# gsgen3d/gsgen

Measured on AMD Instinct MI355X. Metric: fwd+bwd renders/sec (800x800, 100k Gaussians), higher is better.
Workload: dtype f32

## Files before the change

gsgen_amd/csrc/geometry.hip:

```cpp
#include <string.h>

#include "common.hpp"
#include "../../include/gsgen_hip.h"

namespace gs {

constexpr int kThreads = 256;

__device__ __forceinline__ bool sphere_in_frustum(float mx, float my, float mz, float r,
                                                  const float *__restrict__ normal,
                                                  const float *__restrict__ pts) {
  bool ok = true;
#pragma unroll
  for (int k = 0; k < 6; ++k) {
    const float d = (mx - pts[3 * k]) * normal[3 * k] + (my - pts[3 * k + 1]) * normal[3 * k + 1] +
                    (mz - pts[3 * k + 2]) * normal[3 * k + 2];
    ok = ok && (d > -r);
  }
  return ok;
}

__global__ void __launch_bounds__(kThreads)
k_cull_bsphere(uint32_t N, const float *__restrict__ mean, const float *__restrict__ svec,
               const float *__restrict__ normal, const float *__restrict__ pts,
               uint8_t *__restrict__ mask, float thresh) {
  const uint32_t i = blockIdx.x * blockDim.x + threadIdx.x;
  if (i >= N) return;
  const float r = fmaxf(fmaxf(svec[3 * i], svec[3 * i + 1]), svec[3 * i + 2]) * thresh;
  mask[i] = sphere_in_frustum(mean[3 * i], mean[3 * i + 1], mean[3 * i + 2], r, normal, pts) ? 1 : 0;
}

struct Proj {
  float m2x, m2y, c00, c01, c10, c11, depth;
  float A[9];
};

__device__ __forceinline__ void quat_to_rot(const float *__restrict__ q, float *R) {
  float n = sqrtf(q[0] * q[0] + q[1] * q[1] + q[2] * q[2] + q[3] * q[3]);
  n = fmaxf(n, 1e-12f);
  const float w = q[0] / n, x = q[1] / n, y = q[2] / n, z = q[3] / n;
  const float tx = 2.0f * x, ty = 2.0f * y, tz = 2.0f * z;
  const float twx = tx * w, twy = ty * w, twz = tz * w;
  const float txx = tx * x, txy = ty * x, txz = tz * x;
  const float tyy = ty * y, tyz = tz * y, tzz = tz * z;
  R[0] = 1.0f - (tyy + tzz); R[1] = txy - twz;          R[2] = txz + twy;
  R[3] = txy + twz;          R[4] = 1.0f - (txx + tzz); R[5] = tyz - twx;
  R[6] = txz - twy;          R[7] = tyz + twx;          R[8] = 1.0f - (txx + tyy);
}

__device__ __forceinline__ Proj project_one(const float *__restrict__ p, const float *__restrict__ q,
                                            const float *__restrict__ s, const float *Rc,
                                            const float *t) {
  Proj o;
  const float d0 = p[0] - t[0], d1 = p[1] - t[1], d2 = p[2] - t[2];
  float u[3];
#pragma unroll
  for (int i = 0; i < 3; ++i) u[i] = Rc[i] * d0 + Rc[3 + i] * d1 + Rc[6 + i] * d2;
  float Rq[9];
  quat_to_rot(q, Rq);
  float M[9];
#pragma unroll
  for (int i = 0; i < 3; ++i)
#pragma unroll
    for (int j = 0; j < 3; ++j) M[i * 3 + j] = s[j] * Rq[i * 3 + j];
  float S[9];
#pragma unroll
  for (int i = 0; i < 3; ++i)
#pragma unroll
    for (int k = 0; k < 3; ++k)
      S[i * 3 + k] = M[i * 3] * M[k * 3] + M[i * 3 + 1] * M[k * 3 + 1] + M[i * 3 + 2] * M[k * 3 + 2];
  const float x = u[0], y = u[1], z = u[2];
  const float l = sqrtf(x * x + y * y + z * z);
  const float J[9] = {1.0f / z, 0.0f, -x / z / z, 0.0f, 1.0f / z, -y / z / z, x / l, y / l, z / l};
#pragma unroll
  for (int i = 0; i < 3; ++i)
#pragma unroll
    for (int k = 0; k < 3; ++k)
      o.A[i * 3 + k] = J[i * 3] * Rc[k * 3] + J[i * 3 + 1] * Rc[k * 3 + 1] + J[i * 3 + 2] * Rc[k * 3 + 2];
  float T1[6];
#pragma unroll
  for (int a = 0; a < 2; ++a)
#pragma unroll
    for (int k = 0; k < 3; ++k)
      T1[a * 3 + k] = o.A[a * 3] * S[k] + o.A[a * 3 + 1] * S[3 + k] + o.A[a * 3 + 2] * S[6 + k];
  o.c00 = T1[0] * o.A[0] + T1[1] * o.A[1] + T1[2] * o.A[2];
  o.c01 = T1[0] * o.A[3] + T1[1] * o.A[4] + T1[2] * o.A[5];
  o.c10 = T1[3] * o.A[0] + T1[4] * o.A[1] + T1[5] * o.A[2];
  o.c11 = T1[3] * o.A[3] + T1[4] * o.A[4] + T1[5] * o.A[5];
  o.depth = z;
  o.m2x = x / z;
  o.m2y = y / z;
  return o;
}

__device__ __forceinline__ void load_pose(const float *__restrict__ c2w, float *Rc, float *t) {
#pragma unroll
  for (int i = 0; i < 3; ++i) {
#pragma unroll
    for (int j = 0; j < 3; ++j) Rc[i * 3 + j] = c2w[i * 4 + j];
    t[i] = c2w[i * 4 + 3];
  }
}

__global__ void __launch_bounds__(kThreads)
k_project(uint32_t N, const float *__restrict__ mean, const float *__restrict__ qvec,
          const float *__restrict__ svec, const float *__restrict__ c2w, float *__restrict__ mean2d,
          float *__restrict__ cov2d, float *__restrict__ JW, float *__restrict__ depth) {
  const uint32_t i = blockIdx.x * blockDim.x + threadIdx.x;
  if (i >= N) return;
  float Rc[9], t[3];
  load_pose(c2w, Rc, t);
  const Proj o = project_one(mean + 3 * (size_t)i, qvec + 4 * (size_t)i, svec + 3 * (size_t)i, Rc, t);
  *reinterpret_cast<float2 *>(mean2d + 2 * (size_t)i) = make_float2(o.m2x, o.m2y);
  *reinterpret_cast<float4 *>(cov2d + 4 * (size_t)i) = make_float4(o.c00, o.c01, o.c10, o.c11);
  depth[i] = o.depth;
  if (JW != nullptr) {
#pragma unroll
    for (int k = 0; k < 9; ++k) JW[9 * (size_t)i + k] = o.A[k];
  }
}

constexpr int kAdamMaxGroups = 8;
struct AdamArgs {
  uint64_t end[kAdamMaxGroups];
  float step_size[kAdamMaxGroups];
  uint32_t n_groups;
  float bc2_sqrt, beta1, beta2, eps;
  const float *dev;
};

__global__ void __launch_bounds__(kThreads)
k_adam_step(uint64_t n, float *__restrict__ param, const float *__restrict__ grad,
            float *__restrict__ exp_avg, float *__restrict__ exp_avg_sq, AdamArgs a) {
  const uint64_t i0 = 4 * ((uint64_t)blockIdx.x * blockDim.x + threadIdx.x);
  if (i0 >= n) return;
  const float w1 = 1.0f - a.beta1, w2 = 1.0f - a.beta2;
  if (a.dev != nullptr) {
#pragma unroll
    for (int k = 0; k < kAdamMaxGroups; ++k) a.step_size[k] = a.dev[k];
    a.bc2_sqrt = a.dev[kAdamMaxGroups];
  }
#pragma unroll
  for (int e = 0; e < 4; ++e) {
    const uint64_t i = i0 + e;
    if (i >= n) break;
    float ss = a.step_size[0];
#pragma unroll
    for (int k = 1; k < kAdamMaxGroups; ++k)
      if (k < (int)a.n_groups && i >= a.end[k - 1]) ss = a.step_size[k];
    const float g = grad[i];
    float m = exp_avg[i], v = exp_avg_sq[i];
    m = m + (g - m) * w1;
    v = v * a.beta2 + (w2 * g) * g;
    const float denom = sqrtf(v) / a.bc2_sqrt + a.eps;
    param[i] = param[i] - ss * (m / denom);
    exp_avg[i] = m;
    exp_avg_sq[i] = v;
  }
}

__global__ void __launch_bounds__(kThreads)
k_densify_update(uint32_t N, const float *__restrict__ cov2d, const float *__restrict__ g_mean2d,
                 const uint8_t *__restrict__ mask, float *__restrict__ max_radii2d,
                 float *__restrict__ grad_accum, float *__restrict__ cnt) {
  const uint32_t n = blockIdx.x * blockDim.x + threadIdx.x;
  if (n >= N) return;
  if (mask != nullptr && mask[n] == 0) return;
  if (max_radii2d != nullptr) {
    const float4 c = *reinterpret_cast<const float4 *>(cov2d + 4 * (size_t)n);
    const float m = (c.x + c.w) / 2.0f;
    const float det = c.x * c.w - c.y * c.z;
    const float r = m + sqrtf(fmaxf(m * m - det, 0.0f));
    if (!(r < 0.0f)) atomicMax(reinterpret_cast<unsigned int *>(max_radii2d) + n, __float_as_uint(r));
  }
  if (grad_accum != nullptr) {
    const float2 g = *reinterpret_cast<const float2 *>(g_mean2d + 2 * (size_t)n);
    atomicAdd(grad_accum + n, sqrtf(g.x * g.x + g.y * g.y));
    if (cnt != nullptr) atomicAdd(cnt + n, 1.0f);
  }
}

constexpr int kStatViews = 16;
struct DensifyViews {
  const float *cov2d[kStatViews], *g_mean2d[kStatViews];
  const uint8_t *mask[kStatViews];
};
__global__ void __launch_bounds__(kThreads)
k_densify_update_views(uint32_t N, DensifyViews dv, int n_views, float *__restrict__ max_radii2d,
                       float *__restrict__ grad_accum, float *__restrict__ cnt) {
  const uint32_t n = blockIdx.x * blockDim.x + threadIdx.x;
  if (n >= N) return;
  float rmax = 0.0f, gsum = 0.0f, visits = 0.0f;
  bool seen = false, rnan = false;
  for (int v = 0; v < n_views; ++v) {
    const uint8_t *m = dv.mask[v];
    if (m != nullptr && m[n] == 0) continue;
    seen = true;
    if (max_radii2d != nullptr) {
      const float4 c = *reinterpret_cast<const float4 *>(dv.cov2d[v] + 4 * (size_t)n);
      const float mm = (c.x + c.w) / 2.0f;
      const float det = c.x * c.w - c.y * c.z;
      const float r = mm + sqrtf(fmaxf(mm * mm - det, 0.0f));
      if (r != r) rnan = true;
      else rmax = fmaxf(rmax, r);
    }
    if (grad_accum != nullptr) {
      const float2 g = *reinterpret_cast<const float2 *>(dv.g_mean2d[v] + 2 * (size_t)n);
      gsum += sqrtf(g.x * g.x + g.y * g.y);
      visits += 1.0f;
    }
  }
  if (!seen) return;
  if (max_radii2d != nullptr)
    atomicMax(reinterpret_cast<unsigned int *>(max_radii2d) + n,
              rnan ? 0x7fc00000u : __float_as_uint(rmax));
  if (grad_accum != nullptr) {
    atomicAdd(grad_accum + n, gsum);
    if (cnt != nullptr) atomicAdd(cnt + n, visits);
  }
}

struct ProjGrad { float gm[3], gq[4], gs[3]; };
struct CholK { double k0, k1, k2; };
__device__ __forceinline__ CholK chol_k_of(const float *__restrict__ cov2d_n) {
  const CholRec c = chol_prep(cov2d_n[0], cov2d_n[1], cov2d_n[2], cov2d_n[3]);
  CholK k{0.0, 0.0, 0.0};
  if (c.ok) { k.k0 = (double)kInvSc2 * (double)c.p0; k.k1 = (double)kInvSc2 * (double)c.p1; k.k2 = (double)kInvSc2 * (double)c.p2; }
  return k;
}
__device__ __forceinline__ ProjGrad project_bwd_one(uint32_t n, const float *__restrict__ mean,
                                                    const float *__restrict__ qvec, const float *__restrict__ svec,
                                                    const float *__restrict__ c2w, int detach_depth,
                                                    double gm0, double gm1, const double (&gc)[4], float g_depth_n) {
#pragma clang fp contract(fast)
  ProjGrad o;
  double Rc[9], t[3];
#pragma unroll
  for (int i = 0; i < 3; ++i) {
#pragma unroll
    for (int j = 0; j < 3; ++j) Rc[i * 3 + j] = (double)c2w[i * 4 + j];
    t[i] = (double)c2w[i * 4 + 3];
  }
  const float *p = mean + 3 * (size_t)n, *q = qvec + 4 * (size_t)n, *sf = svec + 3 * (size_t)n;
  const double s[3] = {(double)sf[0], (double)sf[1], (double)sf[2]};
  const double d0 = (double)p[0] - t[0], d1 = (double)p[1] - t[1], d2 = (double)p[2] - t[2];
  double u[3];
#pragma unroll
  for (int i = 0; i < 3; ++i) u[i] = Rc[i] * d0 + Rc[3 + i] * d1 + Rc[6 + i] * d2;
  double nq = sqrt((double)q[0] * q[0] + (double)q[1] * q[1] + (double)q[2] * q[2] + (double)q[3] * q[3]);
  nq = nq < 1e-12 ? 1e-12 : nq;
  const double inq = 1.0 / nq;
  const double w = q[0] * inq, x = q[1] * inq, y = q[2] * inq, z = q[3] * inq;
  const double Rq[9] = {1 - 2 * (y * y + z * z), 2 * (x * y - w * z), 2 * (x * z + w * y),
                        2 * (x * y + w * z), 1 - 2 * (x * x + z * z), 2 * (y * z - w * x),
                        2 * (x * z - w * y), 2 * (y * z + w * x), 1 - 2 * (x * x + y * y)};
  double M[9];
#pragma unroll
  for (int i = 0; i < 3; ++i)
#pragma unroll
    for (int j = 0; j < 3; ++j) M[i * 3 + j] = s[j] * Rq[i * 3 + j];
  const double ux = u[0], uy = u[1], uz = u[2];
  const double iz = 1.0 / uz;
  const double j02 = -ux * iz * iz, j12 = -uy * iz * iz;
  double A[6];
#pragma unroll
  for (int k = 0; k < 3; ++k) {
    A[k] = iz * Rc[k * 3] + j02 * Rc[k * 3 + 2];
    A[3 + k] = iz * Rc[k * 3 + 1] + j12 * Rc[k * 3 + 2];
  }
  double GA[6];
#pragma unroll
  for (int k = 0; k < 3; ++k) {
    GA[k] = gc[0] * A[k] + gc[1] * A[3 + k];
    GA[3 + k] = gc[2] * A[k] + gc[3] * A[3 + k];
  }
  double dS[9];
#pragma unroll
  for (int j = 0; j < 3; ++j)
#pragma unroll
    for (int k = 0; k < 3; ++k) dS[j * 3 + k] = A[j] * GA[k] + A[3 + j] * GA[3 + k];
  double dM[9];
#pragma unroll
  for (int i = 0; i < 3; ++i)
#pragma unroll
    for (int j = 0; j < 3; ++j) {
      double acc = 0.0;
#pragma unroll
      for (int k = 0; k < 3; ++k) acc += (dS[i * 3 + k] + dS[k * 3 + i]) * M[k * 3 + j];
      dM[i * 3 + j] = acc;
    }
  double dR[9];
#pragma unroll
  for (int j = 0; j < 3; ++j) {
    double acc = 0.0;
#pragma unroll
    for (int i = 0; i < 3; ++i) {
      acc += dM[i * 3 + j] * Rq[i * 3 + j];
      dR[i * 3 + j] = dM[i * 3 + j] * s[j];
    }
    o.gs[j] = (float)acc;
  }
  double dq[4];
  dq[0] = 2 * (-z * dR[1] + y * dR[2] + z * dR[3] - x * dR[5] - y * dR[6] + x * dR[7]);
  dq[1] = 2 * (y * dR[1] + z * dR[2] + y * dR[3] - 2 * x * dR[4] - w * dR[5] + z * dR[6] + w * dR[7] - 2 * x * dR[8]);
  dq[2] = 2 * (-2 * y * dR[0] + x * dR[1] + w * dR[2] + x * dR[3] + z * dR[5] - w * dR[6] + z * dR[7] - 2 * y * dR[8]);
  dq[3] = 2 * (-2 * z * dR[0] - w * dR[1] + x * dR[2] + w * dR[3] - 2 * z * dR[4] + y * dR[5] + x * dR[6] + y * dR[7]);
  const double qh[4] = {w, x, y, z};
  const double dot = qh[0] * dq[0] + qh[1] * dq[1] + qh[2] * dq[2] + qh[3] * dq[3];
#pragma unroll
  for (int k = 0; k < 4; ++k) o.gq[k] = (float)((dq[k] - qh[k] * dot) * inq);
  double du[3] = {gm0 * iz, gm1 * iz, (double)g_depth_n};
  if (!detach_depth) du[2] += -(ux * gm0 + uy * gm1) * iz * iz;
#pragma unroll
  for (int j = 0; j < 3; ++j) o.gm[j] = (float)(Rc[j * 3] * du[0] + Rc[j * 3 + 1] * du[1] + Rc[j * 3 + 2] * du[2]);
  return o;
}
__device__ __forceinline__ ProjGrad project_bwd_one(uint32_t n, const float *__restrict__ mean,
                                                    const float *__restrict__ qvec, const float *__restrict__ svec,
                                                    const float *__restrict__ c2w, int detach_depth,
                                                    const float *__restrict__ g_mean2d,
                                                    const float *__restrict__ g_cov2d, float g_depth_n) {
  const float4 g = *reinterpret_cast<const float4 *>(g_cov2d + 4 * (size_t)n);
  const double gc[4] = {(double)g.x, (double)g.y, (double)g.z, (double)g.w};
  return project_bwd_one(n, mean, qvec, svec, c2w, detach_depth, (double)g_mean2d[2 * (size_t)n],
                         (double)g_mean2d[2 * (size_t)n + 1], gc, g_depth_n);
}

template <bool ACC>
__global__ void __launch_bounds__(kThreads)
k_project_bwd(uint32_t N, const float *__restrict__ mean, const float *__restrict__ qvec,
              const float *__restrict__ svec, const float *__restrict__ c2w, int detach_depth,
              const uint8_t *__restrict__ mask, const float *__restrict__ g_mean2d,
              const float *__restrict__ g_cov2d, const float *__restrict__ g_depth,
              float *__restrict__ g_mean, float *__restrict__ g_qvec, float *__restrict__ g_svec) {
  const uint32_t n = blockIdx.x * blockDim.x + threadIdx.x;
  if (n >= N) return;
  float *gm = g_mean + 3 * (size_t)n, *gq = g_qvec + 4 * (size_t)n, *gs_ = g_svec + 3 * (size_t)n;
  if (mask != nullptr && mask[n] == 0) {
    if constexpr (!ACC) {
      gm[0] = gm[1] = gm[2] = 0.f;
      gq[0] = gq[1] = gq[2] = gq[3] = 0.f;
      gs_[0] = gs_[1] = gs_[2] = 0.f;
    }
    return;
  }
  auto put = [](float *dst, float v) {
    if constexpr (ACC) atomicAdd(dst, v);
    else *dst = v;
  };
  const ProjGrad o = project_bwd_one(n, mean, qvec, svec, c2w, detach_depth, g_mean2d, g_cov2d,
                                     g_depth != nullptr ? g_depth[n] : 0.0f);
#pragma unroll
  for (int j = 0; j < 3; ++j) put(gs_ + j, o.gs[j]);
#pragma unroll
  for (int k = 0; k < 4; ++k) put(gq + k, o.gq[k]);
#pragma unroll
  for (int j = 0; j < 3; ++j) put(gm + j, o.gm[j]);
}

constexpr int kProjViews = 16;
struct ProjBwdViews {
  const float *cam[kProjViews];
  const uint8_t *mask[kProjViews];
  const float *g_mean2d[kProjViews], *g_cov2d[kProjViews], *g_depth[kProjViews];
  const float *g_chan6[kProjViews], *depth[kProjViews];
  const float *cov2d[kProjViews];
  const float *chol[kProjViews];
};
__device__ __forceinline__ void moments_to_grads(const CholK &k, const float *__restrict__ mom2, const float *__restrict__ mom4,
                                                 double &gm0, double &gm1, double (&gc)[4]) {
  const double Mu = (double)mom2[0], Mv = (double)mom2[1];
  const double Muu = (double)mom4[0], Muv = (double)mom4[1], Mvv = (double)mom4[2];
  gm0 = k.k0 * Mu;
  gm1 = k.k1 * Mu + k.k2 * Mv;
  gc[0] = 0.5 * k.k0 * k.k0 * Muu;
  gc[1] = gc[2] = 0.5 * k.k0 * (k.k1 * Muu + k.k2 * Muv);
  gc[3] = 0.5 * (k.k1 * k.k1 * Muu + 2.0 * k.k1 * k.k2 * Muv + k.k2 * k.k2 * Mvv);
}
__device__ __forceinline__ void moments_to_grads_sh(const float *__restrict__ cov2d_n, const float *__restrict__ mom2,
                                                    const float *__restrict__ mom4, double &gm0, double &gm1, double (&gc)[4]) {
  const float det = cov2d_n[0] * cov2d_n[3] - cov2d_n[1] * cov2d_n[2];
  const bool ok = (det > 0.0f) && (fabsf(det) <= 3.402823466e+38f);
  const double inv = ok ? 1.0 / (double)det : 0.0;
  const double h = 0.5 * inv * inv;
  gm0 = inv * (double)mom2[0];
  gm1 = inv * (double)mom2[1];
  gc[0] = h * (double)mom4[0];
  gc[1] = gc[2] = h * (double)mom4[1];
  gc[3] = h * (double)mom4[2];
}
constexpr int kPbvThreads = 128;
constexpr int kPbvGauss = 64, kPbvLanes = kPbvThreads / kPbvGauss;
__global__ void __launch_bounds__(kPbvThreads)
k_project_bwd_views(uint32_t N, const float *__restrict__ mean, const float *__restrict__ qvec,
                    const float *__restrict__ svec, ProjBwdViews pv, int n_views, int detach_depth, int accumulate,
                    int moments, float *__restrict__ g_mean, float *__restrict__ g_qvec, float *__restrict__ g_svec,
                    float *__restrict__ g_color, float *__restrict__ stat_accum, float *__restrict__ stat_cnt) {
  __shared__ float part[kPbvLanes > 1 ? kPbvLanes - 1 : 1][15][kPbvGauss];
  const int gl = (int)(threadIdx.x & (kPbvGauss - 1)), vq = (int)(threadIdx.x / kPbvGauss);
  const uint32_t n = blockIdx.x * kPbvGauss + gl;
  const bool live = n < N;
  ProjGrad a;
  float gc[3] = {0.f, 0.f, 0.f};
  float gsum = 0.f, visits = 0.f;
#pragma unroll
  for (int j = 0; j < 3; ++j) { a.gm[j] = 0.f; a.gs[j] = 0.f; }
#pragma unroll
  for (int k = 0; k < 4; ++k) a.gq[k] = 0.f;
  if (live) {
    for (int v = vq; v < n_views; v += kPbvLanes) {
      const uint8_t *m = pv.mask[v];
      if (m != nullptr && m[n] == 0) continue;
      const float *ch = pv.g_chan6[v];
      float gd = pv.g_depth[v] != nullptr ? pv.g_depth[v][n] : 0.f;
      if (ch != nullptr) {
        const float2 *c2 = reinterpret_cast<const float2 *>(ch + 6 * (size_t)n);
        const float2 c01 = c2[0], c23 = c2[1], c45 = c2[2];
        gc[0] += c01.x; gc[1] += c01.y; gc[2] += c23.x;
        gd = c23.y + 2.0f * pv.depth[v][n] * c45.y;
      }
      ProjGrad o;
      if (moments) {
        double gm0, gm1, gcv[4];
        if (moments == 2)
          moments_to_grads_sh(pv.cov2d[v] + 4 * (size_t)n, pv.g_mean2d[v] + 2 * (size_t)n, pv.g_cov2d[v] + 4 * (size_t)n, gm0, gm1, gcv);
        else {
          CholK ck;
          if (pv.chol[v] != nullptr) {
            const float4 c = *reinterpret_cast<const float4 *>(pv.chol[v] + 4 * (size_t)n);
            const double on = c.w != 0.0f ? (double)kInvSc2 : 0.0;
            ck = CholK{on * (double)c.x, on * (double)c.y, on * (double)c.z};
          } else {
            ck = chol_k_of(pv.cov2d[v] + 4 * (size_t)n);
          }
          moments_to_grads(ck, pv.g_mean2d[v] + 2 * (size_t)n, pv.g_cov2d[v] + 4 * (size_t)n, gm0, gm1, gcv);
        }
        *reinterpret_cast<float2 *>(const_cast<float *>(pv.g_mean2d[v]) + 2 * (size_t)n) = make_float2((float)gm0, (float)gm1);
        if (stat_accum != nullptr) {
          const float gx = (float)gm0, gy = (float)gm1;
          gsum += sqrtf(gx * gx + gy * gy);
          visits += 1.0f;
        }
        o = project_bwd_one(n, mean, qvec, svec, pv.cam[v], detach_depth, gm0, gm1, gcv, gd);
      } else {
        if (stat_accum != nullptr) {
          const float2 g2 = *reinterpret_cast<const float2 *>(pv.g_mean2d[v] + 2 * (size_t)n);
          gsum += sqrtf(g2.x * g2.x + g2.y * g2.y);
          visits += 1.0f;
        }
        o = project_bwd_one(n, mean, qvec, svec, pv.cam[v], detach_depth, pv.g_mean2d[v], pv.g_cov2d[v], gd);
      }
#pragma unroll
      for (int j = 0; j < 3; ++j) { a.gm[j] += o.gm[j]; a.gs[j] += o.gs[j]; }
#pragma unroll
      for (int k = 0; k < 4; ++k) a.gq[k] += o.gq[k];
    }
  }
  if (vq > 0) {
    float (*mine)[kPbvGauss] = part[vq - 1];
#pragma unroll
    for (int j = 0; j < 3; ++j) { mine[j][gl] = a.gm[j]; mine[3 + j][gl] = a.gs[j]; mine[10 + j][gl] = gc[j]; }
#pragma unroll
    for (int k = 0; k < 4; ++k) mine[6 + k][gl] = a.gq[k];
    mine[13][gl] = gsum; mine[14][gl] = visits;
  }
  __syncthreads();
  if (vq > 0 || !live) return;
  float *gm = g_mean + 3 * (size_t)n, *gq = g_qvec + 4 * (size_t)n, *gs_ = g_svec + 3 * (size_t)n;
  float *gc_ = g_color != nullptr ? g_color + 3 * (size_t)n : nullptr;
#pragma unroll
  for (int q = 0; q < kPbvLanes - 1; ++q) {
#pragma unroll
    for (int j = 0; j < 3; ++j) { a.gm[j] += part[q][j][gl]; a.gs[j] += part[q][3 + j][gl]; gc[j] += part[q][10 + j][gl]; }
#pragma unroll
    for (int k = 0; k < 4; ++k) a.gq[k] += part[q][6 + k][gl];
    gsum += part[q][13][gl]; visits += part[q][14][gl];
  }
  if (stat_accum != nullptr && visits > 0.0f) {
    atomicAdd(stat_accum + n, gsum);
    if (stat_cnt != nullptr) atomicAdd(stat_cnt + n, visits);
  }
  if (accumulate) {
#pragma unroll
    for (int j = 0; j < 3; ++j) { a.gm[j] += gm[j]; a.gs[j] += gs_[j]; if (gc_ != nullptr) gc[j] += gc_[j]; }
#pragma unroll
    for (int k = 0; k < 4; ++k) a.gq[k] += gq[k];
  }
#pragma unroll
  for (int j = 0; j < 3; ++j) { gm[j] = a.gm[j]; gs_[j] = a.gs[j]; }
#pragma unroll
  for (int k = 0; k < 4; ++k) gq[k] = a.gq[k];
  if (gc_ != nullptr) { gc_[0] = gc[0]; gc_[1] = gc[1]; gc_[2] = gc[2]; }
}

__device__ __forceinline__ int to_i32_trunc(float v) {
  if (!(v == v) || v >= 2147483648.0f || v <= -2147483904.0f) return (int)0x80000000;
  return (int)v;
}
__device__ __forceinline__ int clampi(int v, int lo, int hi) { return v < lo ? lo : (v > hi ? hi : v); }

struct Rect { int x0, y0, x1, y1; };
__device__ __forceinline__ Rect tile_rect(float m2x, float m2y, float c00, float c11, float Dr,
                                          float fx, float fy, float cx, float cy, int w, int h, int shift = 4, int side = 0) {
  const float ax = sqrtf(Dr * c00), ay = sqrtf(Dr * c11);
  const float tlx = m2x - ax, tly = m2y - ay, brx = m2x + ax, bry = m2y + ay;
  float m;
  m = tlx * fx; int px0 = to_i32_trunc(m + cx);
  m = tly * fy; int py0 = to_i32_trunc(m + cy);
  m = brx * fx; int px1 = to_i32_trunc(m + cx);
  m = bry * fy; int py1 = to_i32_trunc(m + cy);
  px0 = clampi(px0, 0, w - 1); px1 = clampi(px1, 0, w - 1);
  py0 = clampi(py0, 0, h - 1); py1 = clampi(py1, 0, h - 1);
  Rect r;
  if (side > 0) { r.x0 = px0 / side; r.y0 = py0 / side; r.x1 = px1 / side; r.y1 = py1 / side; return r; }
  r.x0 = px0 >> shift; r.y0 = py0 >> shift; r.x1 = px1 >> shift; r.y1 = py1 >> shift;
  return r;
}

__global__ void __launch_bounds__(kThreads)
k_aabb_count(uint32_t N, const float *__restrict__ mean2d, const float *__restrict__ cov2d,
             float fx, float fy, float cx, float cy, int w, int h, float Dr, int shift, int side,
             int *__restrict__ tl, int *__restrict__ br, uint32_t *__restrict__ total) {
  const uint32_t i = blockIdx.x * blockDim.x + threadIdx.x;
  uint32_t cnt = 0;
  if (i < N) {
    const float2 m = *reinterpret_cast<const float2 *>(mean2d + 2 * (size_t)i);
    const float4 c = *reinterpret_cast<const float4 *>(cov2d + 4 * (size_t)i);
    const Rect r = tile_rect(m.x, m.y, c.x, c.w, Dr, fx, fy, cx, cy, w, h, shift, side);
    *reinterpret_cast<int2 *>(tl + 2 * (size_t)i) = make_int2(r.x0, r.y0);
    *reinterpret_cast<int2 *>(br + 2 * (size_t)i) = make_int2(r.x1, r.y1);
    cnt = (uint32_t)((r.x1 - r.x0 + 1) * (r.y1 - r.y0 + 1));
  }
  float dummy = 0.f; (void)dummy;
  uint32_t s = cnt;
#pragma unroll
  for (int m = 32; m >= 1; m >>= 1) s += (uint32_t)__shfl_xor((int)s, m, 64);
  if ((threadIdx.x & 63u) == 0 && s != 0) atomicAdd(total, s);
}

__device__ __forceinline__ void
frame_project_body(uint32_t N, const float *__restrict__ mean, const float *__restrict__ qvec,
                const float *__restrict__ svec, const float *__restrict__ cam, int w, int h, int ntw,
                float *__restrict__ mean2d, float *__restrict__ cov2d, float *__restrict__ depth,
                uint8_t *__restrict__ mask, int *__restrict__ tl, int *__restrict__ br, float *__restrict__ chol = nullptr,
                float *__restrict__ max_radii2d = nullptr) {
  const uint32_t i = blockIdx.x * blockDim.x + threadIdx.x;
  if (i >= N) return;
  float Rc[9], t[3];
  load_pose(cam, Rc, t);
  const float fx = cam[12], fy = cam[13], cx = cam[14], cy = cam[15];
  const float frustum_r = cam[16], Dr = cam[17];
  const float *p = mean + 3 * (size_t)i, *s = svec + 3 * (size_t)i;
  bool in = true;
  if (frustum_r > 0.0f) {
    const float r = fmaxf(fmaxf(s[0], s[1]), s[2]) * frustum_r;
    in = sphere_in_frustum(p[0], p[1], p[2], r, cam + 20, cam + 38);
  }
  Rect rc{0, 0, -1, -1};
  float2 m2 = make_float2(0.f, 0.f);
  float4 c2 = make_float4(1.f, 0.f, 0.f, 1.f);
  float z = 0.f;
  if (in) {
    const Proj o = project_one(p, qvec + 4 * (size_t)i, s, Rc, t);
    m2 = make_float2(o.m2x, o.m2y);
    c2 = make_float4(o.c00, o.c01, o.c10, o.c11);
    z = o.depth;
    rc = tile_rect(o.m2x, o.m2y, o.c00, o.c11, Dr, fx, fy, cx, cy, w, h);
  }
  *reinterpret_cast<float2 *>(mean2d + 2 * (size_t)i) = m2;
  *reinterpret_cast<float4 *>(cov2d + 4 * (size_t)i) = c2;
  if (chol != nullptr) {
    const CholRec c = chol_prep(c2.x, c2.y, c2.z, c2.w);
    *reinterpret_cast<float4 *>(chol + 4 * (size_t)i) = make_float4(c.p0, c.p1, c.p2, (in && c.ok) ? 1.0f : 0.0f);
  }
  if (max_radii2d != nullptr && in) {
    const float mm = (c2.x + c2.w) / 2.0f;
    const float det = c2.x * c2.w - c2.y * c2.z;
    const float r = mm + sqrtf(fmaxf(mm * mm - det, 0.0f));
    if (r != r) atomicMax(reinterpret_cast<unsigned int *>(max_radii2d) + i, 0x7fc00000u);
    else if (!(r < 0.0f)) atomicMax(reinterpret_cast<unsigned int *>(max_radii2d) + i, __float_as_uint(r));
  }
  depth[i] = z;
  mask[i] = in ? 1 : 0;
  *reinterpret_cast<int2 *>(tl + 2 * (size_t)i) = make_int2(rc.x0, rc.y0);
  *reinterpret_cast<int2 *>(br + 2 * (size_t)i) = make_int2(rc.x1, rc.y1);
  (void)ntw;
}

__global__ void __launch_bounds__(kThreads)
k_frame_project(uint32_t N, const float *__restrict__ mean, const float *__restrict__ qvec,
                const float *__restrict__ svec, const float *__restrict__ cam, int w, int h, int ntw,
                float *__restrict__ mean2d, float *__restrict__ cov2d, float *__restrict__ depth,
                uint8_t *__restrict__ mask, int *__restrict__ tl, int *__restrict__ br) {
  frame_project_body(N, mean, qvec, svec, cam, w, h, ntw, mean2d, cov2d, depth, mask, tl, br);
}
constexpr int kViewPack = 8;
struct GeoViewPack { GeoView v[kViewPack]; };
constexpr int kFrameThreads = 256;
__global__ void __launch_bounds__(kFrameThreads)
k_frame_project_views(uint32_t N, const float *__restrict__ mean, const float *__restrict__ qvec,
                      const float *__restrict__ svec, int w, int h, int ntw, GeoViewPack pack, GeoView *__restrict__ dst,
                      float4 *__restrict__ z_shared, uint32_t z_quads) {
  const GeoView &v = pack.v[blockIdx.y];
  if (blockIdx.x == 0 && threadIdx.x == 0) dst[blockIdx.y] = v;
  if (z_shared != nullptr) {
    const uint32_t nthr = gridDim.x * gridDim.y * blockDim.x;
    for (uint32_t i = (blockIdx.y * gridDim.x + blockIdx.x) * blockDim.x + threadIdx.x; i < z_quads; i += nthr)
      z_shared[i] = make_float4(0.f, 0.f, 0.f, 0.f);
  }
  const uint32_t i = blockIdx.x * blockDim.x + threadIdx.x;
  if (i < N) {
    if (v.z_mean2d != nullptr) *reinterpret_cast<float2 *>(v.z_mean2d + 2 * (size_t)i) = make_float2(0.f, 0.f);
    if (v.z_cov2d != nullptr) *reinterpret_cast<float4 *>(v.z_cov2d + 4 * (size_t)i) = make_float4(0.f, 0.f, 0.f, 0.f);
    if (v.z_chan6 != nullptr) {
      float2 *z = reinterpret_cast<float2 *>(v.z_chan6 + 6 * (size_t)i);
      z[0] = z[1] = z[2] = make_float2(0.f, 0.f);
    }
  }
  frame_project_body(N, mean, qvec, svec, v.cam, w, h, ntw, v.mean2d, v.cov2d, v.depth, v.mask, v.tl, v.br, v.chol, v.max_r);
}

static inline dim3 grid_for(uint32_t n) { return dim3((n + kThreads - 1) / kThreads); }

}

using namespace gs;

namespace gs {
constexpr float kMinScale = 1e-3f;
__device__ __forceinline__ float act_fwd(int code, float x) {
  switch (code) {
    case 1: return expf(x);
    case 2: return 1.0f / (1.0f + expf(-x));
    case 3: return fabsf(x);
    case 4: return fmaxf(x, 0.0f);
    case 5: return x > 20.0f ? x : log1pf(expf(x));
    case 6: return fmaxf(x, 0.0f) + kMinScale;
    case 7: return fabsf(x) + kMinScale;
    default: return x;
  }
}
__device__ __forceinline__ float act_bwd(int code, float x, float y) {
  switch (code) {
    case 1: return y;
    case 2: return y * (1.0f - y);
    case 3: case 7: return x > 0.0f ? 1.0f : (x < 0.0f ? -1.0f : 0.0f);
    case 4: case 6: return x > 0.0f ? 1.0f : 0.0f;
    case 5: return x > 20.0f ? 1.0f : 1.0f / (1.0f + expf(-x));
    default: return 1.0f;
  }
}
__global__ void __launch_bounds__(kThreads)
k_activate_fields(uint32_t N, const float *__restrict__ svec_raw, const float *__restrict__ alpha_raw,
                  const float *__restrict__ color_raw, int sa, int aa, int ca, float *__restrict__ svec, float *__restrict__ alpha,
                  float *__restrict__ color) {
  const uint32_t i = blockIdx.x * blockDim.x + threadIdx.x;
  if (i >= 3 * N) return;
  svec[i] = act_fwd(sa, svec_raw[i]);
  color[i] = act_fwd(ca, color_raw[i]);
  if (i < N) alpha[i] = act_fwd(aa, alpha_raw[i]);
}
__global__ void __launch_bounds__(kThreads)
k_activate_fields_bwd(uint32_t N, const float *__restrict__ svec_raw, const float *__restrict__ alpha_raw,
                      const float *__restrict__ color_raw, const float *__restrict__ svec, const float *__restrict__ alpha,
                      const float *__restrict__ color, int sa, int aa, int ca, float *__restrict__ g_svec, float *__restrict__ g_alpha,
                      float *__restrict__ g_color) {
  const uint32_t i = blockIdx.x * blockDim.x + threadIdx.x;
  if (i >= 3 * N) return;
  g_svec[i] *= act_bwd(sa, svec_raw[i], svec[i]);
  g_color[i] *= act_bwd(ca, color_raw[i], color[i]);
  if (i < N) g_alpha[i] *= act_bwd(aa, alpha_raw[i], alpha[i]);
}
}
extern "C" int gsgen_activate_fields(uint32_t N, const float *svec_raw, const float *alpha_raw, const float *color_raw,
                                     int svec_act, int alpha_act, int color_act, float *svec, float *alpha, float *color,
                                     gsgen_stream_t stream) {
  if (N == 0) return 0;
  if (!svec_raw || !alpha_raw || !color_raw || !svec || !alpha || !color) return GSGEN_EINVAL;
  if (svec_act < 0 || svec_act > 7 || alpha_act < 0 || alpha_act > 7 || color_act < 0 || color_act > 7) return GSGEN_EUNSUPPORTED;
  hipLaunchKernelGGL(gs::k_activate_fields, gs::grid_for(3 * N), dim3(gs::kThreads), 0, (hipStream_t)stream, N, svec_raw, alpha_raw,
                     color_raw, svec_act, alpha_act, color_act, svec, alpha, color);
  return (int)hipGetLastError();
}
extern "C" int gsgen_activate_fields_backward(uint32_t N, const float *svec_raw, const float *alpha_raw, const float *color_raw,
                                              const float *svec, const float *alpha, const float *color, int svec_act,
                                              int alpha_act, int color_act, float *g_svec, float *g_alpha, float *g_color,
                                              gsgen_stream_t stream) {
  if (N == 0) return 0;
  if (!svec_raw || !alpha_raw || !color_raw || !svec || !alpha || !color || !g_svec || !g_alpha || !g_color) return GSGEN_EINVAL;
  if (svec_act < 0 || svec_act > 7 || alpha_act < 0 || alpha_act > 7 || color_act < 0 || color_act > 7) return GSGEN_EUNSUPPORTED;
  hipLaunchKernelGGL(gs::k_activate_fields_bwd, gs::grid_for(3 * N), dim3(gs::kThreads), 0, (hipStream_t)stream, N, svec_raw, alpha_raw,
                     color_raw, svec, alpha, color, svec_act, alpha_act, color_act, g_svec, g_alpha, g_color);
  return (int)hipGetLastError();
}

namespace gs {
constexpr int kUploadWords = 896;
struct UploadPack { uint32_t w[kUploadWords]; };
__global__ void __launch_bounds__(256) k_upload_words(UploadPack pack, uint32_t *dst, int n) {
  for (int i = (int)threadIdx.x; i < n; i += (int)blockDim.x) dst[i] = pack.w[i];
}
}

extern "C" int gsgen_upload_small(void *dst, const void *host_src, size_t bytes, gsgen_stream_t stream) {
  if (bytes == 0) return 0;
  if (!dst || !host_src || (bytes & 3u) != 0 || (reinterpret_cast<uintptr_t>(dst) & 3u) != 0) return GSGEN_EINVAL;
  const uint32_t *src = static_cast<const uint32_t *>(host_src);
  uint32_t *d = static_cast<uint32_t *>(dst);
  size_t words = bytes / 4;
  while (words > 0) {
    const int n = (int)(words < (size_t)gs::kUploadWords ? words : (size_t)gs::kUploadWords);
    gs::UploadPack pack;
    memcpy(pack.w, src, (size_t)n * 4);
    hipLaunchKernelGGL(gs::k_upload_words, dim3(1), dim3(256), 0, (hipStream_t)stream, pack, d, n);
    src += n; d += n; words -= (size_t)n;
  }
  return (int)hipGetLastError();
}

extern "C" {

int gsgen_culling_gaussian_bsphere(uint32_t N, const float *mean, const float *qvec,
                                   const float *svec, const float *normal, const float *pts,
                                   uint8_t *mask, float thresh, gsgen_stream_t stream) {
  (void)qvec;
  if (N == 0) return 0;
  if (!mean || !svec || !normal || !pts || !mask) return GSGEN_EINVAL;
  hipLaunchKernelGGL(k_cull_bsphere, grid_for(N), dim3(kThreads), 0, (hipStream_t)stream, N, mean,
                     svec, normal, pts, mask, thresh);
  return (int)hipGetLastError();
}

int gsgen_project_gaussians(uint32_t N, const float *mean, const float *qvec, const float *svec,
                            const float *c2w, float *mean2d, float *cov2d, float *JW, float *depth,
                            gsgen_stream_t stream) {
  if (N == 0) return 0;
  if (!mean || !qvec || !svec || !c2w || !mean2d || !cov2d || !depth) return GSGEN_EINVAL;
  hipLaunchKernelGGL(k_project, grid_for(N), dim3(kThreads), 0, (hipStream_t)stream, N, mean, qvec,
                     svec, c2w, mean2d, cov2d, JW, depth);
  return (int)hipGetLastError();
}

int gsgen_project_gaussians_backward_masked(uint32_t N, const float *mean, const float *qvec,
                                            const float *svec, const float *c2w, int detach_depth,
                                            const uint8_t *mask, const float *g_mean2d,
                                            const float *g_cov2d, const float *g_depth,
                                            float *g_mean, float *g_qvec, float *g_svec,
                                            gsgen_stream_t stream) {
  if (N == 0) return 0;
  if (!mean || !qvec || !svec || !c2w || !g_mean2d || !g_cov2d || !g_mean || !g_qvec || !g_svec)
    return GSGEN_EINVAL;
  hipLaunchKernelGGL(k_project_bwd<false>, grid_for(N), dim3(kThreads), 0, (hipStream_t)stream, N,
                     mean, qvec, svec, c2w, detach_depth, mask, g_mean2d, g_cov2d, g_depth, g_mean,
                     g_qvec, g_svec);
  return (int)hipGetLastError();
}

int gsgen_project_gaussians_backward_accum(uint32_t N, const float *mean, const float *qvec,
                                           const float *svec, const float *c2w, int detach_depth,
                                           const uint8_t *mask, const float *g_mean2d,
                                           const float *g_cov2d, const float *g_depth,
                                           float *g_mean, float *g_qvec, float *g_svec,
                                           gsgen_stream_t stream) {
  if (N == 0) return 0;
  if (!mean || !qvec || !svec || !c2w || !g_mean2d || !g_cov2d || !g_mean || !g_qvec || !g_svec)
    return GSGEN_EINVAL;
  hipLaunchKernelGGL(k_project_bwd<true>, grid_for(N), dim3(kThreads), 0, (hipStream_t)stream, N,
                     mean, qvec, svec, c2w, detach_depth, mask, g_mean2d, g_cov2d, g_depth, g_mean,
                     g_qvec, g_svec);
  return (int)hipGetLastError();
}

static int project_bwd_batch(uint32_t n_views, uint32_t N, const float *mean, const float *qvec, const float *svec,
                             const float *const *c2w, int detach_depth, const uint8_t *const *mask,
                             const float *const *g_mean2d, const float *const *g_cov2d, const float *const *g_depth,
                             const float *const *g_chan6, const float *const *depth, float *g_mean, float *g_qvec,
                             float *g_svec, float *g_color, gsgen_stream_t stream, const float *const *cov2d = nullptr,
                             int moments_form = 1, const float *const *chol = nullptr, float *stat_accum = nullptr,
                             float *stat_cnt = nullptr) {
  if (N == 0) return 0;
  if (!mean || !qvec || !svec || !g_mean || !g_qvec || !g_svec) return GSGEN_EINVAL;
  if (n_views && (!c2w || !g_mean2d || !g_cov2d)) return GSGEN_EINVAL;
  if ((g_chan6 != nullptr) != (depth != nullptr) || (g_chan6 != nullptr) != (g_color != nullptr)) return GSGEN_EINVAL;
  for (uint32_t v = 0; v < n_views; ++v) {
    if (!c2w[v] || !g_mean2d[v] || !g_cov2d[v]) return GSGEN_EINVAL;
    if (g_chan6 && (!g_chan6[v] || !depth[v])) return GSGEN_EINVAL;
    if (cov2d && !cov2d[v]) return GSGEN_EINVAL;
  }
  uint32_t v0 = 0;
  do {
    ProjBwdViews pv{};
    const uint32_t nv = (n_views - v0) < (uint32_t)kProjViews ? (n_views - v0) : (uint32_t)kProjViews;
    for (uint32_t i = 0; i < nv; ++i) {
      pv.cam[i] = c2w[v0 + i];
// ... 274 lines not shown
```

Measured before the change: 7474.

## Accumulate symmetric covariance gradient across views before quaternion/scale backprop

The projection backward pass now splits into a per-Gaussian prologue (quaternion normalisation, rotation matrix, scaled M), a per-view step that only accumulates a symmetric 6-entry world-space covariance gradient and the mean gradient, and a single tail that backpropagates through M, R and q once per Gaussian instead of once per view. Camera matrices are converted to double once into shared memory, and the cross-lane reduction now passes double partial sums for S and gm. This removes the repeated per-view double-precision rotation and quaternion chain, at the cost of more shared memory and double-typed partials. A side effect is that visits is now counted regardless of stat_accum, and Gaussians with no visits get zeroed outputs.

```diff
diff --git a/gsgen_amd/csrc/geometry.hip b/gsgen_amd/csrc/geometry.hip
--- a/gsgen_amd/csrc/geometry.hip
+++ b/gsgen_amd/csrc/geometry.hip
@@ -228,57 +228,83 @@
   if (c.ok) { k.k0 = (double)kInvSc2 * (double)c.p0; k.k1 = (double)kInvSc2 * (double)c.p1; k.k2 = (double)kInvSc2 * (double)c.p2; }
   return k;
 }
-__device__ __forceinline__ ProjGrad project_bwd_one(uint32_t n, const float *__restrict__ mean,
-                                                    const float *__restrict__ qvec, const float *__restrict__ svec,
-                                                    const float *__restrict__ c2w, int detach_depth,
-                                                    double gm0, double gm1, const double (&gc)[4], float g_depth_n) {
+struct ProjPre { double s[3], qh[4], inq, Rq[9], M[9]; };
+struct ProjSum { double S[6], gm[3]; };
+__device__ __forceinline__ ProjPre project_bwd_pre(const float *__restrict__ q, const float *__restrict__ sf) {
 #pragma clang fp contract(fast)
-  ProjGrad o;
-  double Rc[9], t[3];
-#pragma unroll
-  for (int i = 0; i < 3; ++i) {
-#pragma unroll
-    for (int j = 0; j < 3; ++j) Rc[i * 3 + j] = (double)c2w[i * 4 + j];
-    t[i] = (double)c2w[i * 4 + 3];
-  }
-  const float *p = mean + 3 * (size_t)n, *q = qvec + 4 * (size_t)n, *sf = svec + 3 * (size_t)n;
-  const double s[3] = {(double)sf[0], (double)sf[1], (double)sf[2]};
-  const double d0 = (double)p[0] - t[0], d1 = (double)p[1] - t[1], d2 = (double)p[2] - t[2];
-  double u[3];
-#pragma unroll
-  for (int i = 0; i < 3; ++i) u[i] = Rc[i] * d0 + Rc[3 + i] * d1 + Rc[6 + i] * d2;
+  ProjPre g;
+#pragma unroll
+  for (int j = 0; j < 3; ++j) g.s[j] = (double)sf[j];
   double nq = sqrt((double)q[0] * q[0] + (double)q[1] * q[1] + (double)q[2] * q[2] + (double)q[3] * q[3]);
   nq = nq < 1e-12 ? 1e-12 : nq;
-  const double inq = 1.0 / nq;
-  const double w = q[0] * inq, x = q[1] * inq, y = q[2] * inq, z = q[3] * inq;
+  g.inq = 1.0 / nq;
+  const double w = q[0] * g.inq, x = q[1] * g.inq, y = q[2] * g.inq, z = q[3] * g.inq;
+  g.qh[0] = w; g.qh[1] = x; g.qh[2] = y; g.qh[3] = z;
   const double Rq[9] = {1 - 2 * (y * y + z * z), 2 * (x * y - w * z), 2 * (x * z + w * y),
                         2 * (x * y + w * z), 1 - 2 * (x * x + z * z), 2 * (y * z - w * x),
                         2 * (x * z - w * y), 2 * (y * z + w * x), 1 - 2 * (x * x + y * y)};
-  double M[9];
 #pragma unroll
   for (int i = 0; i < 3; ++i)
 #pragma unroll
-    for (int j = 0; j < 3; ++j) M[i * 3 + j] = s[j] * Rq[i * 3 + j];
-  const double ux = u[0], uy = u[1], uz = u[2];
-  const double iz = 1.0 / uz;
-  const double j02 = -ux * iz * iz, j12 = -uy * iz * iz;
-  double A[6];
+    for (int j = 0; j < 3; ++j) { g.Rq[i * 3 + j] = Rq[i * 3 + j]; g.M[i * 3 + j] = g.s[j] * Rq[i * 3 + j]; }
+  return g;
+}
+__device__ __forceinline__ void project_bwd_view(const double (&p)[3], const double *__restrict__ cam, int detach_depth, double gm0,
+                                                 double gm1, const double (&gc)[4], float g_depth_n, ProjSum &a) {
+#pragma clang fp contract(fast)
+  double Rc[9];
+#pragma unroll
+  for (int i = 0; i < 3; ++i)
+#pragma unroll
+    for (int j = 0; j < 3; ++j) Rc[i * 3 + j] = cam[i * 4 + j];
+  const double d0 = p[0] - cam[3], d1 = p[1] - cam[7], d2 = p[2] - cam[11];
+  double u[3];
+#pragma unroll
+  for (int i = 0; i < 3; ++i) u[i] = Rc[i] * d0 + Rc[3 + i] * d1 + Rc[6 + i] * d2;
+  const double iz = 1.0 / u[2];
+  const double a0 = -u[0] * iz, a1 = -u[1] * iz;
+  double B[6];
 #pragma unroll
   for (int k = 0; k < 3; ++k) {
-    A[k] = iz * Rc[k * 3] + j02 * Rc[k * 3 + 2];
-    A[3 + k] = iz * Rc[k * 3 + 1] + j12 * Rc[k * 3 + 2];
-  }
-  double GA[6];
+    B[k] = Rc[k * 3] + a0 * Rc[k * 3 + 2];
+    B[3 + k] = Rc[k * 3 + 1] + a1 * Rc[k * 3 + 2];
+  }
+  const double iz2 = iz * iz;
+  const double h00 = iz2 * (gc[0] + gc[0]), h01 = iz2 * (gc[1] + gc[2]), h11 = iz2 * (gc[3] + gc[3]);
+  double HB[6];
 #pragma unroll
   for (int k = 0; k < 3; ++k) {
-    GA[k] = gc[0] * A[k] + gc[1] * A[3 + k];
-    GA[3 + k] = gc[2] * A[k] + gc[3] * A[3 + k];
-  }
-  double dS[9];
+    HB[k] = h00 * B[k] + h01 * B[3 + k];
+    HB[3 + k] = h01 * B[k] + h11 * B[3 + k];
+  }
+  int e = 0;
 #pragma unroll
   for (int j = 0; j < 3; ++j)
 #pragma unroll
-    for (int k = 0; k < 3; ++k) dS[j * 3 + k] = A[j] * GA[k] + A[3 + j] * GA[3 + k];
+    for (int k = j; k < 3; ++k, ++e) {
+      a.S[e] += B[j] * HB[k];
+      a.S[e] += B[3 + j] * HB[3 + k];
+    }
+  double du[3] = {gm0 * iz, gm1 * iz, (double)g_depth_n};
+  if (!detach_depth) du[2] += (a0 * gm0 + a1 * gm1) * iz;
+#pragma unroll
+  for (int j = 0; j < 3; ++j) {
+    a.gm[j] += Rc[j * 3] * du[0];
+    a.gm[j] += Rc[j * 3 + 1] * du[1];
+    a.gm[j] += Rc[j * 3 + 2] * du[2];
+  }
+}
+__device__ __forceinline__ void project_bwd_view(uint32_t n, const double (&p)[3], const double *__restrict__ cam, int detach_depth,
+                                                 const float *__restrict__ g_mean2d, const float *__restrict__ g_cov2d,
+                                                 float g_depth_n, ProjSum &a) {
+  const float4 g = *reinterpret_cast<const float4 *>(g_cov2d + 4 * (size_t)n);
+  const double gc[4] = {(double)g.x, (double)g.y, (double)g.z, (double)g.w};
+  project_bwd_view(p, cam, detach_depth, (double)g_mean2d[2 * (size_t)n], (double)g_mean2d[2 * (size_t)n + 1], gc, g_depth_n, a);
+}
+__device__ __forceinline__ ProjGrad project_bwd_tail(const ProjPre &g, const ProjSum &a) {
+#pragma clang fp contract(fast)
+  ProjGrad o;
+  const double Ss[9] = {a.S[0], a.S[1], a.S[2], a.S[1], a.S[3], a.S[4], a.S[2], a.S[4], a.S[5]};
   double dM[9];
 #pragma unroll
   for (int i = 0; i < 3; ++i)
@@ -286,7 +312,7 @@
     for (int j = 0; j < 3; ++j) {
       double acc = 0.0;
 #pragma unroll
-      for (int k = 0; k < 3; ++k) acc += (dS[i * 3 + k] + dS[k * 3 + i]) * M[k * 3 + j];
+      for (int k = 0; k < 3; ++k) acc += Ss[i * 3 + k] * g.M[k * 3 + j];
       dM[i * 3 + j] = acc;
     }
   double dR[9];
@@ -295,35 +321,27 @@
     double acc = 0.0;
 #pragma unroll
     for (int i = 0; i < 3; ++i) {
-      acc += dM[i * 3 + j] * Rq[i * 3 + j];
-      dR[i * 3 + j] = dM[i * 3 + j] * s[j];
+      acc += dM[i * 3 + j] * g.Rq[i * 3 + j];
+      dR[i * 3 + j] = dM[i * 3 + j] * g.s[j];
     }
     o.gs[j] = (float)acc;
   }
+  const double w = g.qh[0], x = g.qh[1], y = g.qh[2], z = g.qh[3];
   double dq[4];
   dq[0] = 2 * (-z * dR[1] + y * dR[2] + z * dR[3] - x * dR[5] - y * dR[6] + x * dR[7]);
   dq[1] = 2 * (y * dR[1] + z * dR[2] + y * dR[3] - 2 * x * dR[4] - w * dR[5] + z * dR[6] + w * dR[7] - 2 * x * dR[8]);
   dq[2] = 2 * (-2 * y * dR[0] + x * dR[1] + w * dR[2] + x * dR[3] + z * dR[5] - w * dR[6] + z * dR[7] - 2 * y * dR[8]);
   dq[3] = 2 * (-2 * z * dR[0] - w * dR[1] + x * dR[2] + w * dR[3] - 2 * z * dR[4] + y * dR[5] + x * dR[6] + y * dR[7]);
-  const double qh[4] = {w, x, y, z};
-  const double dot = qh[0] * dq[0] + qh[1] * dq[1] + qh[2] * dq[2] + qh[3] * dq[3];
-#pragma unroll
-  for (int k = 0; k < 4; ++k) o.gq[k] = (float)((dq[k] - qh[k] * dot) * inq);
-  double du[3] = {gm0 * iz, gm1 * iz, (double)g_depth_n};
-  if (!detach_depth) du[2] += -(ux * gm0 + uy * gm1) * iz * iz;
-#pragma unroll
-  for (int j = 0; j < 3; ++j) o.gm[j] = (float)(Rc[j * 3] * du[0] + Rc[j * 3 + 1] * du[1] + Rc[j * 3 + 2] * du[2]);
+  const double dot = g.qh[0] * dq[0] + g.qh[1] * dq[1] + g.qh[2] * dq[2] + g.qh[3] * dq[3];
+#pragma unroll
+  for (int k = 0; k < 4; ++k) o.gq[k] = (float)((dq[k] - g.qh[k] * dot) * g.inq);
+#pragma unroll
+  for (int j = 0; j < 3; ++j) o.gm[j] = (float)a.gm[j];
   return o;
 }
-__device__ __forceinline__ ProjGrad project_bwd_one(uint32_t n, const float *__restrict__ mean,
-                                                    const float *__restrict__ qvec, const float *__restrict__ svec,
-                                                    const float *__restrict__ c2w, int detach_depth,
-                                                    const float *__restrict__ g_mean2d,
-                                                    const float *__restrict__ g_cov2d, float g_depth_n) {
-  const float4 g = *reinterpret_cast<const float4 *>(g_cov2d + 4 * (size_t)n);
-  const double gc[4] = {(double)g.x, (double)g.y, (double)g.z, (double)g.w};
-  return project_bwd_one(n, mean, qvec, svec, c2w, detach_depth, (double)g_mean2d[2 * (size_t)n],
-                         (double)g_mean2d[2 * (size_t)n + 1], gc, g_depth_n);
+__device__ __forceinline__ void load_mean_f64(const float *__restrict__ mean, uint32_t n, double (&p)[3]) {
+  const float *m = mean + 3 * (size_t)n;
+  p[0] = (double)m[0]; p[1] = (double)m[1]; p[2] = (double)m[2];
 }
 
 template <bool ACC>
@@ -348,8 +366,14 @@
     if constexpr (ACC) atomicAdd(dst, v);
     else *dst = v;
   };
-  const ProjGrad o = project_bwd_one(n, mean, qvec, svec, c2w, detach_depth, g_mean2d, g_cov2d,
-                                     g_depth != nullptr ? g_depth[n] : 0.0f);
+  double p[3];
+  load_mean_f64(mean, n, p);
+  double cam[12];
+#pragma unroll
+  for (int i = 0; i < 12; ++i) cam[i] = (double)c2w[i];
+  ProjSum a{};
+  project_bwd_view(n, p, cam, detach_depth, g_mean2d, g_cov2d, g_depth != nullptr ? g_depth[n] : 0.0f, a);
+  const ProjGrad o = project_bwd_tail(project_bwd_pre(qvec + 4 * (size_t)n, svec + 3 * (size_t)n), a);
 #pragma unroll
   for (int j = 0; j < 3; ++j) put(gs_ + j, o.gs[j]);
 #pragma unroll
@@ -396,18 +420,24 @@
                     const float *__restrict__ svec, ProjBwdViews pv, int n_views, int detach_depth, int accumulate,
                     int moments, float *__restrict__ g_mean, float *__restrict__ g_qvec, float *__restrict__ g_svec,
                     float *__restrict__ g_color, float *__restrict__ stat_accum, float *__restrict__ stat_cnt) {
-  __shared__ float part[kPbvLanes > 1 ? kPbvLanes - 1 : 1][15][kPbvGauss];
+  __shared__ double dpart[kPbvLanes > 1 ? kPbvLanes - 1 : 1][9][kPbvGauss];
+  __shared__ float fpart[kPbvLanes > 1 ? kPbvLanes - 1 : 1][5][kPbvGauss];
+  __shared__ double camd[kProjViews][12];
   const int gl = (int)(threadIdx.x & (kPbvGauss - 1)), vq = (int)(threadIdx.x / kPbvGauss);
   const uint32_t n = blockIdx.x * kPbvGauss + gl;
   const bool live = n < N;
-  ProjGrad a;
+  if (threadIdx.x < 12) {
+#pragma unroll
+    for (int v = 0; v < kProjViews; ++v)
+      if (v < n_views) camd[v][threadIdx.x] = (double)pv.cam[v][threadIdx.x];
+  }
+  __syncthreads();
+  ProjSum a{};
   float gc[3] = {0.f, 0.f, 0.f};
   float gsum = 0.f, visits = 0.f;
-#pragma unroll
-  for (int j = 0; j < 3; ++j) { a.gm[j] = 0.f; a.gs[j] = 0.f; }
-#pragma unroll
-  for (int k = 0; k < 4; ++k) a.gq[k] = 0.f;
   if (live) {
+    double p[3];
+    load_mean_f64(mean, n, p);
     for (int v = vq; v < n_views; v += kPbvLanes) {
       const uint8_t *m = pv.mask[v];
       if (m != nullptr && m[n] == 0) continue;
@@ -419,9 +449,9 @@
         gc[0] += c01.x; gc[1] += c01.y; gc[2] += c23.x;
         gd = c23.y + 2.0f * pv.depth[v][n] * c45.y;
       }
-      ProjGrad o;
+      visits += 1.0f;
+      double gm0, gm1, gcv[4];
       if (moments) {
-        double gm0, gm1, gcv[4];
         if (moments == 2)
           moments_to_grads_sh(pv.cov2d[v] + 4 * (size_t)n, pv.g_mean2d[v] + 2 * (size_t)n, pv.g_cov2d[v] + 4 * (size_t)n, gm0, gm1, gcv);
         else {
@@ -436,33 +466,25 @@
           moments_to_grads(ck, pv.g_mean2d[v] + 2 * (size_t)n, pv.g_cov2d[v] + 4 * (size_t)n, gm0, gm1, gcv);
         }
         *reinterpret_cast<float2 *>(const_cast<float *>(pv.g_mean2d[v]) + 2 * (size_t)n) = make_float2((float)gm0, (float)gm1);
-        if (stat_accum != nullptr) {
-          const float gx = (float)gm0, gy = (float)gm1;
-          gsum += sqrtf(gx * gx + gy * gy);
-          visits += 1.0f;
-        }
-        o = project_bwd_one(n, mean, qvec, svec, pv.cam[v], detach_depth, gm0, gm1, gcv, gd);
       } else {
-        if (stat_accum != nullptr) {
-          const float2 g2 = *reinterpret_cast<const float2 *>(pv.g_mean2d[v] + 2 * (size_t)n);
-          gsum += sqrtf(g2.x * g2.x + g2.y * g2.y);
-          visits += 1.0f;
-        }
-        o = project_bwd_one(n, mean, qvec, svec, pv.cam[v], detach_depth, pv.g_mean2d[v], pv.g_cov2d[v], gd);
+        const float2 g2 = *reinterpret_cast<const float2 *>(pv.g_mean2d[v] + 2 * (size_t)n);
+        const float4 g4 = *reinterpret_cast<const float4 *>(pv.g_cov2d[v] + 4 * (size_t)n);
+        gm0 = (double)g2.x; gm1 = (double)g2.y;
+        gcv[0] = (double)g4.x; gcv[1] = (double)g4.y; gcv[2] = (double)g4.z; gcv[3] = (double)g4.w;
       }
-#pragma unroll
-      for (int j = 0; j < 3; ++j) { a.gm[j] += o.gm[j]; a.gs[j] += o.gs[j]; }
-#pragma unroll
-      for (int k = 0; k < 4; ++k) a.gq[k] += o.gq[k];
+      if (stat_accum != nullptr) {
+        const float gx = (float)gm0, gy = (float)gm1;
+        gsum += sqrtf(gx * gx + gy * gy);
+      }
+      project_bwd_view(p, camd[v], detach_depth, gm0, gm1, gcv, gd, a);
     }
   }
   if (vq > 0) {
-    float (*mine)[kPbvGauss] = part[vq - 1];
-#pragma unroll
-    for (int j = 0; j < 3; ++j) { mine[j][gl] = a.gm[j]; mine[3 + j][gl] = a.gs[j]; mine[10 + j][gl] = gc[j]; }
-#pragma unroll
-    for (int k = 0; k < 4; ++k) mine[6 + k][gl] = a.gq[k];
-    mine[13][gl] = gsum; mine[14][gl] = visits;
+#pragma unroll
+    for (int e = 0; e < 6; ++e) dpart[vq - 1][e][gl] = a.S[e];
+#pragma unroll
+    for (int j = 0; j < 3; ++j) { dpart[vq - 1][6 + j][gl] = a.gm[j]; fpart[vq - 1][j][gl] = gc[j]; }
+    fpart[vq - 1][3][gl] = gsum; fpart[vq - 1][4][gl] = visits;
   }
   __syncthreads();
   if (vq > 0 || !live) return;
@@ -471,25 +493,35 @@
 #pragma unroll
   for (int q = 0; q < kPbvLanes - 1; ++q) {
 #pragma unroll
-    for (int j = 0; j < 3; ++j) { a.gm[j] += part[q][j][gl]; a.gs[j] += part[q][3 + j][gl]; gc[j] += part[q][10 + j][gl]; }
-#pragma unroll
-    for (int k = 0; k < 4; ++k) a.gq[k] += part[q][6 + k][gl];
-    gsum += part[q][13][gl]; visits += part[q][14][gl];
-  }
-  if (stat_accum != nullptr && visits > 0.0f) {
+    for (int e = 0; e < 6; ++e) a.S[e] += dpart[q][e][gl];
+#pragma unroll
+    for (int j = 0; j < 3; ++j) { a.gm[j] += dpart[q][6 + j][gl]; gc[j] += fpart[q][j][gl]; }
+    gsum += fpart[q][3][gl]; visits += fpart[q][4][gl];
+  }
+  if (visits == 0.0f) {
+    if (!accumulate) {
+      gm[0] = gm[1] = gm[2] = 0.f;
+      gq[0] = gq[1] = gq[2] = gq[3] = 0.f;
+      gs_[0] = gs_[1] = gs_[2] = 0.f;
+      if (gc_ != nullptr) gc_[0] = gc_[1] = gc_[2] = 0.f;
+    }
+    return;
+  }
+  if (stat_accum != nullptr) {
     atomicAdd(stat_accum + n, gsum);
     if (stat_cnt != nullptr) atomicAdd(stat_cnt + n, visits);
   }
+  ProjGrad o = project_bwd_tail(project_bwd_pre(qvec + 4 * (size_t)n, svec + 3 * (size_t)n), a);
   if (accumulate) {
 #pragma unroll
-    for (int j = 0; j < 3; ++j) { a.gm[j] += gm[j]; a.gs[j] += gs_[j]; if (gc_ != nullptr) gc[j] += gc_[j]; }
-#pragma unroll
-    for (int k = 0; k < 4; ++k) a.gq[k] += gq[k];
-  }
-#pragma unroll
-  for (int j = 0; j < 3; ++j) { gm[j] = a.gm[j]; gs_[j] = a.gs[j]; }
-#pragma unroll
-  for (int k = 0; k < 4; ++k) gq[k] = a.gq[k];
+    for (int j = 0; j < 3; ++j) { o.gm[j] += gm[j]; o.gs[j] += gs_[j]; if (gc_ != nullptr) gc[j] += gc_[j]; }
+#pragma unroll
+    for (int k = 0; k < 4; ++k) o.gq[k] += gq[k];
+  }
+#pragma unroll
+  for (int j = 0; j < 3; ++j) { gm[j] = o.gm[j]; gs_[j] = o.gs[j]; }
+#pragma unroll
+  for (int k = 0; k < 4; ++k) gq[k] = o.gq[k];
   if (gc_ != nullptr) { gc_[0] = gc[0]; gc_[1] = gc[1]; gc_[2] = gc[2]; }
 }
 
```

After: 7527, median of 6. About the same (+0.7%).
